# sahaRatul/sela

Hardware: NVIDIA H100
Metric: encode+decode MSamples/s (higher is better)
Workload: dtype f64+int64

## Files before the change

### sela_b200/csrc/c_abi.cu

```cuda
#include <algorithm>
#include <atomic>
#include <cstdarg>
#include <cstdio>
#include <cstdlib>
#include <cstring>
#include <mutex>
#include <thread>
#include <vector>

#include "lossless.cuh"
#include "verify.cuh"

using namespace selab200;

namespace {

thread_local char g_error[512] = "";
std::mutex g_mutex;
std::atomic<uint64_t> g_launches{0};

int fail(int code, const char *fmt, ...)
{
    va_list ap;
    va_start(ap, fmt);
// ... 217 lines not shown
    const std::pair<const void *, int> key(reinterpret_cast<const void *>(kernel), dev);
    std::lock_guard<std::mutex> lock(m);
    for (auto &e : done)
        if (e.first == key) {
            if (e.second >= bytes)
                return 0;
            CUDA_TRY(cudaFuncSetAttribute(kernel, cudaFuncAttributeMaxDynamicSharedMemorySize, (int)bytes));
            e.second = bytes;
            return 0;
        }
    CUDA_TRY(cudaFuncSetAttribute(kernel, cudaFuncAttributeMaxDynamicSharedMemorySize, (int)bytes));
    done.emplace_back(key, bytes);
    return 0;
}

int launch_check(const char *what)
{
    g_launches.fetch_add(1, std::memory_order_relaxed);
    cudaError_t e = cudaGetLastError();
    if (e != cudaSuccess)
        return fail(SELAB200_ERR_CUDA, "launch of %s failed: %s", what, cudaGetErrorString(e));
    return 0;
}

template <int KIND>
int launch_unit_means(const void *src, size_t n_units, uint32_t channels, double *means, cudaStream_t stream)
{
    const MeanTiling mt = mean_tiling(KIND, channels);
    k_unit_means<KIND><<<(unsigned)((n_units + 31) / 32), 32, unit_means_smem_bytes(mt), stream>>>(src, (uint32_t)n_units,
                                                                                                 channels, means);
    return launch_check("k_unit_means");
}

template <bool STEREO, bool TRACE, bool CHECK = false, bool FORCE = false>
int launch_encode_units(const EncodeParams &p, size_t n_units, selab200_analysis_trace *d_trace, cudaStream_t stream,
                        const selab200_predictor *d_pred = nullptr)
{
    constexpr size_t smem = encode_smem_bytes<STEREO>();
    if (int rc = set_smem(k_encode_units<STEREO, TRACE, CHECK, FORCE>, smem))
        return rc;
    k_encode_units<STEREO, TRACE, CHECK, FORCE><<<(unsigned)n_units, 32, smem, stream>>>(p, d_trace, d_pred);
    return launch_check("k_encode_units");
}

template <bool STEREO, bool FORCE = false>
int launch_repair(const EncodeParams &p, const RepairParams &r, size_t n_frames, size_t n_units, cudaStream_t stream,
                  const selab200_predictor *d_pred = nullptr)
{
    constexpr size_t smem = encode_smem_bytes<STEREO>();
    if (int rc = set_smem(k_lossless_candidates<STEREO, FORCE>, smem))
        return rc;
    if (int rc = set_smem(k_lossless_repack<STEREO, FORCE>, smem))
        return rc;
    k_lossless_select<<<(unsigned)((n_frames + 255) / 256), 256, 0, stream>>>(p, r);
    if (int rc = launch_check("k_lossless_select"))
        return rc;
    const unsigned warps = (unsigned)std::min(n_units, (size_t)g.sms * 32);
    for (int round = 0; round < 2; round++) {
        k_lossless_candidates<STEREO, FORCE><<<warps, 32, smem, stream>>>(p, r, round, d_pred);
        if (int rc = launch_check("k_lossless_candidates"))
            return rc;
    }
    k_lossless_repack<STEREO, FORCE><<<warps, 32, smem, stream>>>(p, r, d_pred);
    if (int rc = launch_check("k_lossless_repack"))
        return rc;
    k_lossless_report<<<(unsigned)std::min((n_frames + 255) / 256, (size_t)g.sms), 256, 0, stream>>>(p, r);
// ... 21 lines not shown

int encode_device(const int16_t *d_pcm, uint32_t n_frames, uint32_t channels, selab200_subframe_desc *d_descs,
                  uint32_t *d_words, size_t capacity, uint64_t *d_used, int32_t *d_status, void *d_ws,
                  size_t ws_bytes, cudaStream_t stream, const EncodeOptions &o = EncodeOptions())
{
    if (int rc = check_channels(channels))
        return rc;
    if (ws_bytes < (o.lossless ? selab200_encode_lossless_workspace_bytes(n_frames, channels)
                               : selab200_encode_workspace_bytes(n_frames, channels)))
        return fail(SELAB200_ERR_ARGUMENT, "encode workspace too small");
    if (channels == 2 && (reinterpret_cast<uintptr_t>(d_pcm) & 15) != 0)
        return fail(SELAB200_ERR_ARGUMENT, "stereo PCM must be 16-byte aligned on the device");
    if (o.fresh) {
        CUDA_TRY(cudaMemsetAsync(d_status, 0, sizeof(int32_t), stream));
        CUDA_TRY(cudaMemsetAsync(d_used, 0, sizeof(uint64_t), stream));
    }
    if (n_frames == 0)
        return 0;
    const bool stereo = channels == 2;
    const size_t n_units = encode_units(n_frames, channels);
    const size_t n_sub = (size_t)n_frames * channels;
    EncodeParams p;
    p.pcm = d_pcm;
    p.n_frames = n_frames;
    p.channels = channels;
    p.descs = d_descs;
    p.words = d_words;
    p.capacity = capacity;
    p.words_used = reinterpret_cast<unsigned long long *>(d_used);
    p.status = d_status;
    p.units = static_cast<UnitRecord *>(d_ws);
    p.slots = reinterpret_cast<uint32_t *>(static_cast<char *>(d_ws) + align256(n_units * sizeof(UnitRecord)));
    p.means = reinterpret_cast<double *>(reinterpret_cast<char *>(p.slots) + align256(n_units * (size_t)kSlotWords * 4));
    p.residues = reinterpret_cast<int32_t *>(reinterpret_cast<char *>(p.means) + align256(n_units * sizeof(double)));
    if (int rc = stereo ? launch_unit_means<kMeanStereo>(d_pcm, n_units, channels, p.means, stream)
                        : launch_unit_means<kMeanPcm>(d_pcm, n_units, channels, p.means, stream))
        return rc;
    if (o.lossless) {
        RepairParams r;
        char *b = static_cast<char *>(d_ws) + align256(selab200_encode_workspace_bytes(n_frames, channels));
        r.count = reinterpret_cast<uint32_t *>(b);
        r.frames = reinterpret_cast<uint32_t *>(b + 256);
        r.orig = reinterpret_cast<UnitRecord *>(b + 256 + align256((size_t)n_frames * 4));
        r.units = reinterpret_cast<RepairUnit *>(reinterpret_cast<char *>(r.orig) + align256(n_units * sizeof(UnitRecord)));
        r.entries = o.lossless->entries;
        r.n_entries = o.lossless->n_entries;
        r.frame_base = o.lossless->frame_base;
        CUDA_TRY(cudaMemsetAsync(r.count, 0, 2 * sizeof(uint32_t), stream));
        if (o.d_pred) {
            if (int rc = stereo ? launch_encode_units<true, false, true, true>(p, n_units, nullptr, stream, o.d_pred)
                                : launch_encode_units<false, false, true, true>(p, n_units, nullptr, stream, o.d_pred))
                return rc;
            if (int rc = stereo ? launch_repair<true, true>(p, r, n_frames, n_units, stream, o.d_pred)
                                : launch_repair<false, true>(p, r, n_frames, n_units, stream, o.d_pred))
                return rc;
        } else {
            if (int rc = stereo ? launch_encode_units<true, false, true>(p, n_units, nullptr, stream)
                                : launch_encode_units<false, false, true>(p, n_units, nullptr, stream))
                return rc;
            if (int rc = stereo ? launch_repair<true>(p, r, n_frames, n_units, stream)
                                : launch_repair<false>(p, r, n_frames, n_units, stream))
                return rc;
        }
    } else {
        const int rc_units = stereo ? (o.d_trace ? launch_encode_units<true, true>(p, n_units, o.d_trace, stream)
                                                 : launch_encode_units<true, false>(p, n_units, nullptr, stream))
                                    : (o.d_trace ? launch_encode_units<false, true>(p, n_units, o.d_trace, stream)
                                                 : launch_encode_units<false, false>(p, n_units, nullptr, stream));
        if (rc_units)
// ... 398 lines not shown
}

void selab200_shutdown(void)
{
    std::lock_guard<std::mutex> lock(g_mutex);
    shutdown_all();
}

void *selab200_host_alloc(size_t bytes)
{
    void *p = nullptr;
    if (cudaMallocHost(&p, bytes ? bytes : 1) != cudaSuccess) {
        fail(SELAB200_ERR_CUDA, "cudaMallocHost(%zu) failed", bytes);
        return nullptr;
    }
    return p;
}

void selab200_host_free(void *p)
{
    if (p)
        cudaFreeHost(p);
}

size_t selab200_encode_words_bound(uint32_t n_frames, uint32_t channels)
{
    return (size_t)n_frames * channels * kSlotWords + 64;
}

size_t selab200_encode_workspace_bytes(uint32_t n_frames, uint32_t channels)
{
    const size_t n_units = encode_units(n_frames, channels);
    return align256(n_units * sizeof(UnitRecord)) + align256(n_units * (size_t)kSlotWords * 4) +
           align256(n_units * sizeof(double)) + n_units * (size_t)kFrame * 4 + 256;
}

size_t selab200_encode_lossless_workspace_bytes(uint32_t n_frames, uint32_t channels)
{
    return align256(selab200_encode_workspace_bytes(n_frames, channels)) + repair_lists_bytes(n_frames, channels);
}

size_t selab200_decode_workspace_bytes(uint32_t n_frames, uint32_t channels)
{
    const size_t n_sub = (size_t)n_frames * channels;
    return align256(n_sub * 128 * 4) + align256(n_sub * kFrame * 4) + align256(synthesis_warps(n_sub) * 32 * 4) +
           align256(n_sub * 64) + 256;
}

size_t selab200_verify_workspace_bytes(uint32_t n_frames, uint32_t channels)
{
    return align256(selab200_decode_workspace_bytes(n_frames, channels)) + align256((size_t)n_frames * channels * kFrame * 2);
}

int selab200_encode_frames_device(const int16_t *d_pcm, uint32_t n_frames, uint32_t channels,
                                  selab200_subframe_desc *d_descs, uint32_t *d_words, size_t words_capacity,
                                  uint64_t *d_words_used, int32_t *d_status, void *d_workspace,
                                  size_t workspace_bytes, void *stream)
{
    std::lock_guard<std::mutex> lock(g_mutex);
    if (int rc = d_pcm ? require_ready_for(d_pcm) : require_ready())
        return rc;
    if (!d_pcm || !d_descs || !d_words || !d_words_used || !d_status || !d_workspace)
        return fail(SELAB200_ERR_ARGUMENT, "null device pointer");
    return encode_device(d_pcm, n_frames, channels, d_descs, d_words, words_capacity, d_words_used, d_status,
                         d_workspace, workspace_bytes, (cudaStream_t)stream);
}

// ... 1170 lines not shown
                       int32_t *residues)
{
    std::lock_guard<std::mutex> lock(g_mutex);
    return fir_probe(samples, orders, c, n, wide, residues, nullptr);
}

int selab200_fir_tie_probe(const int32_t *samples, const int32_t *orders, const int64_t *c, uint32_t n, int wide,
                           int32_t *residues, uint8_t *ties)
{
    std::lock_guard<std::mutex> lock(g_mutex);
    if (int rc = require_ready())
        return rc;
    if (!ties)
        return fail(SELAB200_ERR_ARGUMENT, "null pointer");
    return fir_probe(samples, orders, c, n, wide, residues, ties);
}


int selab200_lpc_residues(const int32_t *samples, uint32_t n_sub, uint8_t *order, int32_t *q, int32_t *residues)
{
    std::lock_guard<std::mutex> lock(g_mutex);
    if (int rc = require_ready())
        return rc;
    if (!samples || !order || !q || !residues)
        return fail(SELAB200_ERR_ARGUMENT, "null pointer");
    if (n_sub == 0)
        return 0;
    for (size_t i = 0; i < (size_t)n_sub * kFrame; i++)
        if (samples[i] > 65535 || samples[i] < -65535)
            return fail(SELAB200_ERR_RANGE, "sample %zu = %d outside the 17-bit domain of 16-bit audio", i, samples[i]);
    const size_t sig = (size_t)n_sub * kFrame * 4;
    if (int rc = g.in.ensure(sig)) return rc;
    if (int rc = g.work.ensure(sig)) return rc;
    if (int rc = g.aux.ensure(align256((size_t)n_sub * sizeof(double)) + (size_t)n_sub * kMaxOrder * 4 + n_sub + 256)) return rc;
    double *d_means = static_cast<double *>(g.aux.ptr);
    int32_t *d_q = reinterpret_cast<int32_t *>(static_cast<char *>(g.aux.ptr) + align256((size_t)n_sub * sizeof(double)));
    uint8_t *d_order = reinterpret_cast<uint8_t *>(d_q + (size_t)n_sub * kMaxOrder);
    CUDA_TRY(cudaMemcpyAsync(g.in.ptr, samples, sig, cudaMemcpyHostToDevice, g.stream));
    if (int rc = launch_unit_means<kMeanPlanar>(g.in.ptr, n_sub, 1, d_means, g.stream))
        return rc;
    k_lpc_residues<<<n_sub, 32, 0, g.stream>>>(static_cast<const int32_t *>(g.in.ptr), d_means, n_sub, d_order, d_q,
                                               static_cast<int32_t *>(g.work.ptr));
    if (int rc = launch_check("k_lpc_residues"))
        return rc;
    CUDA_TRY(cudaMemcpyAsync(residues, g.work.ptr, sig, cudaMemcpyDeviceToHost, g.stream));
    CUDA_TRY(cudaMemcpyAsync(q, d_q, (size_t)n_sub * kMaxOrder * 4, cudaMemcpyDeviceToHost, g.stream));
    CUDA_TRY(cudaMemcpyAsync(order, d_order, n_sub, cudaMemcpyDeviceToHost, g.stream));
    CUDA_TRY(cudaStreamSynchronize(g.stream));
    return 0;
}

int selab200_lpc_samples(const int32_t *residues, uint32_t n_sub, const uint8_t *order, const int32_t *q,
                         int32_t *samples)
{
    std::lock_guard<std::mutex> lock(g_mutex);
    if (int rc = require_ready())
        return rc;
    if (!residues || !order || !q || !samples)
        return fail(SELAB200_ERR_ARGUMENT, "null pointer");
    if (n_sub == 0)
        return 0;
    for (uint32_t i = 0; i < n_sub; i++)
        if (order[i] > kMaxOrder)
            return fail(SELAB200_ERR_BITSTREAM, "order[%u] = %u exceeds %d", i, order[i], kMaxOrder);
    const size_t sig = (size_t)n_sub * kFrame * 4;
    if (int rc = g.in.ensure(sig)) return rc;
    if (int rc = g.work.ensure(sig)) return rc;
    if (int rc = g.aux.ensure((size_t)n_sub * kMaxOrder * 4 + n_sub + 256)) return rc;
    int32_t *d_q = static_cast<int32_t *>(g.aux.ptr);
    uint8_t *d_order = reinterpret_cast<uint8_t *>(d_q + (size_t)n_sub * kMaxOrder);
    CUDA_TRY(cudaMemcpyAsync(g.in.ptr, residues, sig, cudaMemcpyHostToDevice, g.stream));
    CUDA_TRY(cudaMemcpyAsync(d_q, q, (size_t)n_sub * kMaxOrder * 4, cudaMemcpyHostToDevice, g.stream));
    CUDA_TRY(cudaMemcpyAsync(d_order, order, n_sub, cudaMemcpyHostToDevice, g.stream));
    k_lpc_samples<<<n_sub, 32, 0, g.stream>>>(static_cast<const int32_t *>(g.in.ptr), n_sub, d_order, d_q,
// ... 81 lines not shown
```

### sela_b200/csrc/kernels.cuh

```cuda
#pragma once

#include "lpc.cuh"
#include "rice.cuh"
#include "rice_vs.cuh"

namespace selab200 {

enum { kMeanPcm = 0, kMeanStereo = 1, kMeanPlanar = 2 };
constexpr int kMeanTile = 64;
constexpr int kMeanSlots = 16;

struct MeanTiling {
    uint32_t units_per_row;
    uint32_t step;
    uint32_t row_stride;
    uint32_t rows_max;
    uint32_t row_words;
};

__host__ __device__ inline MeanTiling mean_tiling(int kind, uint32_t channels)
{
    MeanTiling t;
    uint32_t span = 1;
    if (kind == kMeanPcm) {
// ... 53 lines not shown
        __syncwarp();
#pragma unroll
        for (int s = 0; s < kMeanSlots; s++)
            if (lane + 32 * s < total) {
                staged[soff[s]] = buf[s].x;
                staged[soff[s] + 1] = buf[s].y;
                staged[soff[s] + 2] = buf[s].z;
                staged[soff[s] + 3] = buf[s].w;
            }
        __syncwarp();
        if (t + 1 < kFrame / kMeanTile)
            fetch(t + 1);
#pragma unroll 8
        for (int j = 0; j < kMeanTile; j++) {
            int x;
            if (KIND == kMeanPcm) {
                x = *reinterpret_cast<const int16_t *>(at + j * mt.step);
            } else if (KIND == kMeanStereo) {
                const uint32_t pair = *reinterpret_cast<const uint32_t *>(at + 4 * j);
                const int a = (int)(pair << 16) >> 16, b = (int)pair >> 16;
                x = role == 0 ? a : role == 1 ? b : a - b;
            } else {
                x = *reinterpret_cast<const int32_t *>(at + 4 * j);
            }
            chain.add(x);
        }
    }
    if (u < n_units)
        means[u] = chain.mean();
}

inline size_t unit_means_smem_bytes(const MeanTiling &mt) { return (size_t)mt.rows_max * mt.row_words * 4; }


constexpr uint32_t kSlotWords = 1600;
constexpr uint32_t kSlotReflWords = 32;

struct __align__(16) UnitRecord {
    uint32_t order;
    uint32_t refl_k, refl_words;
    uint32_t res_k, res_words;
    uint32_t flags;
    uint32_t pad[2];
};

struct EncodeParams {
    const int16_t *pcm;
    uint32_t n_frames, channels;
    selab200_subframe_desc *descs;
    uint32_t *words;
    unsigned long long capacity;
    unsigned long long *words_used;
    int32_t *status;
    UnitRecord *units;
    uint32_t *slots;
    double *means;
    int32_t *residues;
};

__host__ __device__ inline uint32_t encode_units(uint32_t n_frames, uint32_t channels)
{
    return channels == 2 ? n_frames * 3u : n_frames * channels;
}

struct PredictorEdit {
    int order, j, delta;
};
__host__ __device__ inline int repair_round1(int o) { return o == 2 ? 5 : 7; }
__host__ __device__ inline int repair_candidates(int o) { return o < 2 ? 0 : 3 * o - 1; }
constexpr int kRepairRound2Max = 3 * kMaxOrder - 1 - 7;
__host__ __device__ inline PredictorEdit repair_edit(int o, int c)
{
    PredictorEdit e{o, 0, 0};
    const int n1 = repair_round1(o);
    if (c < n1) {
        if (c == n1 - 1) {
            e.order = o - 1;
        } else {
            e.j = (c >> 1) < 2 ? (c >> 1) : o - 1;
            e.delta = (c & 1) ? 1 : -1;
        }
        return e;
    }
    c -= n1;
    const int n_edits = o > 3 ? 2 * (o - 3) : 0;
    if (c < n_edits) {
        e.j = 2 + (c >> 1);
        e.delta = (c & 1) ? 1 : -1;
    } else {
        e.order = o - 2 - (c - n_edits);
    }
    return e;
}

struct RepairUnit {
    uint32_t unit, order;
    unsigned long long best;
};
constexpr unsigned long long kNoCandidate = ~0ull;

enum { kUnitEncode = 0, kUnitCheck = 1, kUnitCandidate = 2, kUnitRepack = 3 };

template <bool STEREO, bool TRACE, int MODE, bool FORCE = false>
__device__ __forceinline__ void encode_unit(const EncodeParams &p, selab200_analysis_trace *trace, const uint32_t unit,
                                            RepairUnit *ru, uint32_t cand, const selab200_predictor *pred = nullptr)
{
    constexpr int kRow = kHistoryPad + kFrame;
    constexpr int kLoWords = (kHistoryPad + kFrame) / 32;
    extern __shared__ __align__(16) unsigned char smem_raw[];
    int16_t *s16 = reinterpret_cast<int16_t *>(smem_raw);
    uint32_t *lo_bits = reinterpret_cast<uint32_t *>(smem_raw + kRow * 2);
    constexpr size_t kSigBytes = kRow * 2 + (STEREO ? kLoWords * 4 : 0);
    AnalysisScratch &scratch = *reinterpret_cast<AnalysisScratch *>(smem_raw + kSigBytes);
    static_assert(kCoefAlias + sizeof(CoefSmem) <= sizeof(AnalysisScratch) && kCoefAlias % 16 == 0, "predictor alias");
    CoefSmem &cf = *reinterpret_cast<CoefSmem *>(smem_raw + kSigBytes + kCoefAlias);

    const int lane = lane_id();
    const uint32_t frame = STEREO ? unit / 3 : unit / p.channels;
    const uint32_t role = STEREO ? unit % 3 : unit % p.channels;

    const int16_t *src = p.pcm + (size_t)frame * kFrame * p.channels;
    for (int j = lane; j < kHistoryPad / 2; j += 32)
        reinterpret_cast<uint32_t *>(s16)[j] = 0;
    int16_t *row = s16 + kHistoryPad;
    Signal sig;
    sig.a = row;
    sig.lo = nullptr;
    if (STEREO) {
        const uint4 *src128 = reinterpret_cast<const uint4 *>(src);
        if (role < 2) {
            const uint32_t sel = role ? 0x7632 : 0x5410;
            for (int j = lane; j < kFrame / 4; j += 32) {
                const uint4 v = src128[j];
                reinterpret_cast<uint2 *>(row)[j] = make_uint2(__byte_perm(v.x, v.y, sel), __byte_perm(v.z, v.w, sel));
            }
        } else {
            if (lane < kHistoryPad / 32)
                lo_bits[lane] = 0;
            uint32_t *lo = lo_bits + kHistoryPad / 32;
            for (int it = 0; it < kFrame / 128; it++) {
                const uint4 v = src128[it * 32 + lane];
                const uint32_t pr[4] = {v.x, v.y, v.z, v.w};
                int d[4];
#pragma unroll
                for (int e = 0; e < 4; e++)
                    d[e] = ((int)(pr[e] << 16) >> 16) - ((int)pr[e] >> 16);
                const uint32_t h01 = ((uint32_t)(d[0] >> 1) & 0xffffu) | ((uint32_t)(d[1] >> 1) << 16);
                const uint32_t h23 = ((uint32_t)(d[2] >> 1) & 0xffffu) | ((uint32_t)(d[3] >> 1) << 16);
                reinterpret_cast<uint2 *>(row)[it * 32 + lane] = make_uint2(h01, h23);
                uint32_t nib = (d[0] & 1) | ((d[1] & 1) << 1) | ((d[2] & 1) << 2) | ((d[3] & 1) << 3);
                nib <<= 4 * (lane & 7);
                nib |= __shfl_xor_sync(kFull, nib, 1);
                nib |= __shfl_xor_sync(kFull, nib, 2);
                nib |= __shfl_xor_sync(kFull, nib, 4);
                if ((lane & 7) == 0)
                    lo[it * 4 + (lane >> 3)] = nib;
            }
            sig.lo = lo;
        }
    } else {
        for (int j = lane; j < kFrame; j += 32)
            row[j] = src[(size_t)j * p.channels + role];
    }
    __syncwarp();

    int32_t *res = p.residues + (size_t)(MODE == kUnitEncode || MODE == kUnitCheck ? unit : blockIdx.x) * kFrame;
    warp_autocorrelation(sig, scratch, shfl_d(lane == 0 ? p.means[unit] : 0.0, 0));
    if constexpr (TRACE) {
        selab200_analysis_trace &tr = trace[unit];
        if (lane == 0)
            tr.mean = p.means[unit];
        for (int i = lane; i <= kMaxOrder; i += 32)
            tr.ac[i] = scratch.ac[i];
    }
    warp_schur(scratch);
    int order = warp_order_and_quantise(scratch, cf);
    if constexpr (FORCE) {
        const selab200_predictor &f = pred[unit];
        for (int i = lane; i < kMaxOrder; i += 32)
            cf.q[i] = f.q[i];
        order = f.order;
        __syncwarp();
    }
    if constexpr (MODE == kUnitCandidate || MODE == kUnitRepack) {
        const PredictorEdit e = repair_edit(order, (int)cand);
        if (e.delta) {
            const int v = cf.q[e.j] + e.delta;
            if (v < -64 || v > 63)
                return;
            __syncwarp();
            if (lane == 0)
                cf.q[e.j] = v;
        } else {
            for (int i = e.order + lane; i < order; i += 32)
                cf.q[i] = 0;
        }
        __syncwarp();
        order = e.order;
    }
    warp_coefficients(cf, scratch.t(), order);
    if constexpr (TRACE) {
        selab200_analysis_trace &tr = trace[unit];
        for (int i = lane; i < kMaxOrder; i += 32) {
            tr.k[i] = scratch.kk()[i];
            tr.q[i] = cf.q[i];
        }
        for (int i = lane; i <= kMaxOrder; i += 32)
            tr.c[i] = i == 0 ? 0 : coef_at(cf, i);
        if (lane == 0)
            tr.order = order;
    }
    static_assert(kPlaneBytes <= kCoefAlias, "FIR digit planes");
    uint32_t *planes = reinterpret_cast<uint32_t *>(scratch.ring);
    constexpr bool kCheck = MODE == kUnitCheck || MODE == kUnitCandidate;
    bool tie;
    if (STEREO && role == 2)
        tie = warp_fir_residual<true, kCheck>(sig, cf, order, planes, res);
    else
        tie = warp_fir_residual<false, kCheck>(sig, cf, order, planes, res);

    const RiceChoice cq = warp_rice_choose(cf.q, order);
    const RiceChoice cr = warp_rice_choose(res, kFrame);
    if constexpr (MODE == kUnitCandidate) {
        __syncwarp();
        for (int l = lane; l < kFrame * 4 / 128; l += 32)
            asm volatile("discard.global.L2 [%0], 128;" ::"l"(res + l * 32) : "memory");
        const unsigned long long round = cand >= (uint32_t)repair_round1(ru->order) ? 1ull : 0ull;
        if (lane == 0 && !tie)
            atomicMin(&ru->best, round << 63 | (unsigned long long)(cq.words + cr.words) << 32 | cand);
        return;
    }
    const bool too_large = cq.words > kSlotReflWords || cr.words > kSlotWords - kSlotReflWords;
    uint32_t *slot = p.slots + (size_t)unit * kSlotWords;
    if (!too_large) {
        warp_rice_pack(cf.q, order, cq, slot);
        warp_rice_pack(res, kFrame, cr, slot + kSlotReflWords);
    }
    __syncwarp();
    for (int l = lane; l < kFrame * 4 / 128; l += 32)
        asm volatile("discard.global.L2 [%0], 128;" ::"l"(res + l * 32) : "memory");
    if (lane == 0) {
        UnitRecord u;
        u.order = order;
        u.refl_k = cq.k;
        u.refl_words = cq.words;
        u.res_k = cr.k;
// ... 563 lines not shown
    for (uint32_t pos = 0; pos < ch; pos++)
        any |= fd[pos].subframe_type == 1;
    if (!any || !frame_check(fd, ch, p.n_words))
        return;
    int16_t *out = p.pcm_out + (size_t)frame * kFrame * ch;
    for (uint32_t pos = 0; pos < ch; pos++) {
        const selab200_subframe_desc d = fd[pos];
        if (d.subframe_type != 1)
            continue;
        const int32_t *diff = p.ws_res + ((size_t)frame * ch + pos) * kFrame;
        for (int t = threadIdx.x; t < kFrame; t += blockDim.x)
            out[(size_t)t * ch + d.channel] =
                (int16_t)(uint16_t)((uint32_t)out[(size_t)t * ch + d.parent_channel] - (uint32_t)diff[t]);
    }
}


struct Row17 {
    __align__(16) int16_t a[kHistoryPad + kFrame];
    uint32_t lo[(kHistoryPad + kFrame) / 32];
    __device__ __forceinline__ Signal stage(const int32_t *src)
    {
        const int lane = lane_id();
        for (int i = lane; i < kHistoryPad / 2; i += 32)
            reinterpret_cast<uint32_t *>(a)[i] = 0;
        if (lane < kHistoryPad / 32)
            lo[lane] = 0;
        stage_17bit_row(src, a + kHistoryPad, lo + kHistoryPad / 32);
        __syncwarp();
        return Signal{a + kHistoryPad, lo + kHistoryPad / 32};
    }
};

__global__ void __launch_bounds__(32) k_lpc_residues(const int32_t *samples, const double *means, uint32_t n_sub,
                                                     uint8_t *order_out, int32_t *q_out, int32_t *residues)
{
    __shared__ __align__(16) AnalysisScratch scratch;
    __shared__ __align__(16) CoefSmem cf;
    __shared__ __align__(16) Row17 row;
    const uint32_t sub = blockIdx.x;
    const int lane = lane_id();
    const Signal sig = row.stage(samples + (size_t)sub * kFrame);
    warp_autocorrelation(sig, scratch, means[sub]);
    warp_schur(scratch);
    const int order = warp_order_and_quantise(scratch, cf);
    warp_coefficients(cf, scratch.t(), order);
    warp_fir_residual<true>(sig, cf, order, reinterpret_cast<uint32_t *>(scratch.ring), residues + (size_t)sub * kFrame);
    for (int i = lane; i < kMaxOrder; i += 32)
        q_out[(size_t)sub * kMaxOrder + i] = i < order ? cf.q[i] : 0;
    if (lane == 0)
        order_out[sub] = (uint8_t)order;
}

template <bool CHECK = false>
__global__ void __launch_bounds__(32) k_fir_probe(const int32_t *samples, const int32_t *orders, const long long *c,
                                                  int wide, int32_t *residues, uint8_t *ties)
{
    __shared__ __align__(16) AnalysisScratch scratch;
    __shared__ __align__(16) CoefSmem cf;
    __shared__ __align__(16) Row17 row;
    const uint32_t sub = blockIdx.x;
    const int lane = lane_id();
    const int32_t *src = samples + (size_t)sub * kFrame;
    Signal sig = row.stage(src);
    if (!wide) {
        for (int j = lane; j < kFrame; j += 32)
            row.a[kHistoryPad + j] = (int16_t)src[j];
        sig.lo = nullptr;
    }
    const int order = orders[sub];
    for (int i = lane; i < 112; i += 32) {
        const long long v = i < order ? c[(size_t)sub * (kMaxOrder + 1) + i + 1] : 0;
        cf.clo[i] = (uint32_t)v;
        cf.chi[i] = (int32_t)(v >> 32);
    }
    __syncwarp();
    uint32_t *planes = reinterpret_cast<uint32_t *>(scratch.ring);
    int32_t *res = residues + (size_t)sub * kFrame;
    const bool tie = wide ? warp_fir_residual<true, CHECK>(sig, cf, order, planes, res)
                          : warp_fir_residual<false, CHECK>(sig, cf, order, planes, res);
    if (CHECK && lane == 0)
        ties[sub] = tie;
}

__global__ void __launch_bounds__(32) k_lpc_samples(const int32_t *residues, uint32_t n_sub, const uint8_t *order_in,
                                                    const int32_t *q_in, int32_t *samples)
{
    __shared__ __align__(16) SegSmem sm;
    const uint32_t sub = blockIdx.x;
    const int lane = lane_id();
    const int order = min((int)order_in[sub], kMaxOrder);
    const int n = segment_width(order);
    if (lane == 0) {
        sm.row_res[0] = residues + (size_t)sub * kFrame;
        sm.row_out[0] = samples + (size_t)sub * kFrame;
        sm.row_mode[0] = 2;
    }
    __syncwarp();
    segment_synthesis(sm, 0, lane, n, 0, 1, lane < n ? order : 0, q_in + (size_t)sub * kMaxOrder, 1);
}

__global__ void k_quantise_probe(const double *k, uint32_t n, int32_t *out)
{
    const uint32_t i = blockIdx.x * blockDim.x + threadIdx.x;
    if (i >= n)
        return;
    const double kv = k[i];
    out[4 * (size_t)i + 0] = quantise_reflection(0, kv);
    out[4 * (size_t)i + 1] = quantise_reflection(1, kv);
    out[4 * (size_t)i + 2] = quantise_reflection(2, kv);
// ... 60 lines not shown
```

### sela_b200/csrc/lpc.cuh

```cuda
#pragma once

#include "common.cuh"
#include "lpc_tables.cuh"

namespace selab200 {

struct CoefSmem {
    uint32_t clo[112];
    int32_t  chi[112];
    int32_t  q[104];
};
struct AnalysisScratch {
    double ring[256];
    double ac[128];
    __device__ __forceinline__ double *kk() { return ring; }
    __device__ __forceinline__ double *t() { return ring + 104; }
};
using LpcSmem = AnalysisScratch;
constexpr size_t kCoefAlias = 208 * sizeof(double);

__device__ __forceinline__ long long coef_at(const CoefSmem &cf, int j)
{
    return (long long)(((unsigned long long)(uint32_t)cf.chi[j - 1] << 32) | cf.clo[j - 1]);
}

__device__ __forceinline__ int ring_chunk(int chunk)
{
    chunk &= 127;
    return chunk ^ ((chunk >> 3) & 1);
}
__device__ __forceinline__ int ring_index(int p)
{
    return (ring_chunk(p >> 1) << 1) | (p & 1);
}

__device__ __forceinline__ double sample_to_x(int s)
{
    const double rcp = 1.0 / 32767.0;
    const double a = (double)s;
    const double q0 = __dmul_rn(a, rcp);
    const double r = __fma_rn(-q0, 32767.0, a);
    return __fma_rn(r, rcp, q0);
}
__device__ __forceinline__ double sample_to_x_div(int s) { return ddiv((double)s, 32767.0); }

struct MeanChain {
    double sum = 0.0;
    __device__ __forceinline__ void add(int s) { sum = dadd(sum, sample_to_x(s)); }
    __device__ __forceinline__ double mean() const { return ddiv(sum, (double)kFrame); }
};

template <typename Sig>
__device__ void warp_autocorrelation(const Sig &sig, LpcSmem &sm, const double mean)
{
    const int lane = lane_id();

    {
        double2 *r2 = reinterpret_cast<double2 *>(sm.ring);
        r2[64 + lane] = make_double2(0.0, 0.0);
        r2[96 + lane] = make_double2(0.0, 0.0);
    }
    double acc0 = 0.0, acc1 = 0.0, acc2 = 0.0, acc3 = 0.0;
    double p1 = 0.0, p2 = 0.0, p3 = 0.0;
    const char *ringb = reinterpret_cast<const char *>(sm.ring);
    int own_off[8];
#pragma unroll
    for (int i = 0; i < 8; i++) {
        const int rel = i - lane;
        own_off[i] = 16 * (2 * rel + ((rel >> 2) & 1));
    }

    for (int tile = 0; tile < kFrame / 128; tile++) {
        __syncwarp();
#pragma unroll
        for (int r = 0; r < 4; r++) {
            int j = tile * 128 + r * 32 + lane;
            sm.ring[ring_index(j)] = dsub(sample_to_x(sig.at(j)), mean);
        }
        __syncwarp();
        for (int blk = 0; blk < 4; blk++) {
            const int gb = (tile * 32 + blk * 8) * 32;
            const char *bbase = ringb + (gb & 2047);
#pragma unroll
            for (int i = 0; i < 8; i++) {
                const int oo = (gb + own_off[i]) & 2047;
                const double2 o0 = *reinterpret_cast<const double2 *>(ringb + oo);
                const double2 o1 = *reinterpret_cast<const double2 *>(ringb + (oo ^ 16));
                constexpr int kSw[8] = {0, 0, 0, 0, 16, 16, 16, 16};
                const double2 b0 = *reinterpret_cast<const double2 *>(bbase + ((32 * i) ^ kSw[i]));
                const double2 b1 = *reinterpret_cast<const double2 *>(bbase + ((32 * i + 16) ^ kSw[i]));
                const double c0 = o0.x, c1 = o0.y, c2 = o1.x, c3 = o1.y;
                acc0 = dadd(acc0, dmul(b0.x, c0));
                acc1 = dadd(acc1, dmul(b0.x, p1));
                acc2 = dadd(acc2, dmul(b0.x, p2));
                acc3 = dadd(acc3, dmul(b0.x, p3));
                acc0 = dadd(acc0, dmul(b0.y, c1));
                acc1 = dadd(acc1, dmul(b0.y, c0));
                acc2 = dadd(acc2, dmul(b0.y, p1));
                acc3 = dadd(acc3, dmul(b0.y, p2));
                acc0 = dadd(acc0, dmul(b1.x, c2));
                acc1 = dadd(acc1, dmul(b1.x, c1));
                acc2 = dadd(acc2, dmul(b1.x, c0));
                acc3 = dadd(acc3, dmul(b1.x, p1));
                acc0 = dadd(acc0, dmul(b1.y, c3));
                acc1 = dadd(acc1, dmul(b1.y, c2));
                acc2 = dadd(acc2, dmul(b1.y, c1));
                acc3 = dadd(acc3, dmul(b1.y, c0));
                p1 = c3;
                p2 = c2;
                p3 = c1;
            }
        }
    }
    __syncwarp();
    sm.ac[4 * lane + 0] = acc0;
    sm.ac[4 * lane + 1] = acc1;
    sm.ac[4 * lane + 2] = acc2;
    sm.ac[4 * lane + 3] = acc3;
    __syncwarp();
    const double ac0 = sm.ac[0];
    __syncwarp();
#pragma unroll
    for (int t = 0; t < 4; t++) {
        int i = lane + 32 * t;
        if (i >= 1 && i <= kMaxOrder)
            sm.ac[i] = ddiv(sm.ac[i], ac0);
    }
    if (lane == 0)
        sm.ac[0] = 1.0;
    __syncwarp();
}

__device__ void warp_schur(LpcSmem &sm)
{
    const int lane = lane_id();
    double *kk = sm.kk();
    double g0[4], g1[4];
#pragma unroll
    for (int m = 0; m < 4; m++) {
        int j = 4 * lane + m;
        double v = (j < kMaxOrder) ? sm.ac[j + 1] : 0.0;
        g0[m] = v;
        g1[m] = v;
    }
    double err = sm.ac[0];
    double head = shfl_d(g1[0], 0);
    double k = ddiv(-head, err);
    err = dadd(err, dmul(head, k));
    if (lane == 0)
        kk[0] = k;
    for (int i = 1; i < kMaxOrder; i++) {
        const double kp = k;
        const double nxt = shfl_down_d(g1[0], 1);
        double up[4] = {g1[1], g1[2], g1[3], nxt};
#pragma unroll
        for (int m = 0; m < 4; m++) {
            double n1 = dadd(up[m], dmul(kp, g0[m]));
            double n0 = dadd(dmul(up[m], kp), g0[m]);
            g1[m] = n1;
            g0[m] = n0;
        }
        head = shfl_d(g1[0], 0);
        k = ddiv(-head, err);
        err = dadd(err, dmul(head, k));
        if (lane == 0)
            kk[i] = k;
    }
    __syncwarp();
}


__device__ __forceinline__ bool reflection_significant(double kv) { return fabs(kv) > 0.05; }

__device__ __forceinline__ int quantise_reflection(int i, double kv)
{
    const double sqrt2 = 1.4142135623730950488016887242096;
    double v;
    if (i == 0)
        v = floor(dmul(64.0, dadd(-1.0, dmul(sqrt2, dsqrt(dadd(kv, 1.0))))));
    else if (i == 1)
        v = floor(dmul(64.0, dadd(-1.0, dmul(sqrt2, dsqrt(dadd(-kv, 1.0))))));
    else
        v = floor(dmul(64.0, kv));
    return isnan(v) ? 0 : __double2int_rz(v);
}

__device__ int warp_order_and_quantise(LpcSmem &sm, CoefSmem &cf)
{
    const int lane = lane_id();
    const double *kk = sm.kk();
    int best = -1;
#pragma unroll
    for (int t = 0; t < 4; t++) {
        int i = lane + 32 * t;
        if (i < kMaxOrder && reflection_significant(kk[i]))
            best = i;
    }
    best = __reduce_max_sync(kFull, best);
    const int order = best < 0 ? 1 : best + 1;

#pragma unroll
    for (int t = 0; t < 4; t++) {
        int i = lane + 32 * t;
        if (i < order) {
            cf.q[i] = quantise_reflection(i, kk[i]);
        } else if (i < 104) {
            cf.q[i] = 0;
        }
    }
    __syncwarp();
    return order;
}

__device__ __forceinline__ double dequantise(int i, int q)
{
    int idx = q + 64;
    idx = idx < 0 ? 0 : (idx > 127 ? 127 : idx);
    if (i == 0)
        return __longlong_as_double((long long)selab200_FIRST_BITS[idx]);
    if (i == 1)
        return idx == 0 ? __longlong_as_double((long long)SELAB200_SECOND0_BITS)
                        : -__longlong_as_double((long long)selab200_FIRST_BITS[idx]);
    return (double)(idx - 64) / 64.0;
// ... 5 lines not shown
    for (int i = lane; i < 112; i += 32) {
        cf.clo[i] = 0;
        cf.chi[i] = 0;
    }
    __syncwarp();
    if (order <= 1)
        return;
    for (int i = 0; i < order; i++) {
        const double ki = dequantise(i, cf.q[i]);
        const int half = i >> 1;
        for (int j = lane; j < half; j += 32) {
            double a = t[j];
            double b = t[i - 1 - j];
            t[j] = dadd(a, dmul(ki, b));
            t[i - 1 - j] = dadd(b, dmul(ki, a));
        }
        if (lane == 0) {
            if (i & 1) {
                double mid = t[half];
                t[half] = dadd(mid, dmul(mid, ki));
            }
            t[i] = ki;
        }
        __syncwarp();
    }
    const double scale = 34359738368.0;
    for (int m = lane; m < order; m += 32) {
        const long long v = __double2ll_rz(dmul(scale, -t[m]));
        cf.clo[m] = (uint32_t)v;
        cf.chi[m] = (int32_t)(v >> 32);
    }
    __syncwarp();
}

constexpr int kPlaneWords = 34;
constexpr size_t kPlaneBytes = 8 * kPlaneWords * 4;

__device__ int warp_fir_planes(const CoefSmem &cf, uint32_t *planes)
{
    const unsigned long long H = 0x8080808080808080ull;
    const int lane = lane_id();
    __syncwarp();
    int nd = 0;
    for (int w = lane; w < kPlaneWords; w += 32) {
        unsigned long long e[4];
#pragma unroll
        for (int i = 0; i < 4; i++) {
            const int j = 4 * w + i - 7;
            const unsigned long long c = (j >= 1 && j <= 112) ? (unsigned long long)coef_at(cf, j) : 0ull;
            e[i] = (c + H) ^ H;
            nd = max(nd, (64 - __clzll((long long)e[i]) + 7) >> 3);
        }
#pragma unroll
        for (int p = 0; p < 8; p++) {
            uint32_t v = 0;
#pragma unroll
            for (int i = 0; i < 4; i++)
                v |= (uint32_t)((e[i] >> (8 * p)) & 0xffu) << (8 * i);
            planes[p * kPlaneWords + w] = v;
        }
    }
    __syncwarp();
    return __reduce_max_sync(kFull, nd);
}

__device__ __forceinline__ uint32_t prmt(uint32_t x, uint32_t y, uint32_t sel)
{
    uint32_t d;
    asm("prmt.b32 %0, %1, %2, %3;" : "=r"(d) : "r"(x), "r"(y), "r"(sel));
// ... 301 lines not shown
```

Before: 12910.

## Compute per-unit autocorrelation in a dedicated multi-unit warp kernel

Moves the LPC autocorrelation out of the per-unit encode warp into a new kernel that processes four units per warp, with eight lanes per unit each holding thirteen lag accumulators over a shared-memory sliding window. The normalised autocorrelation is written to a global workspace, and Schur recursion reads it from there. The analysis scratch is also shrunk to a union of kk, t and the FIR planes, plus the coefficient struct, which lowers shared memory per block. The trade-off is an extra kernel launch and a global round trip for the autocorrelation rows, and the FP accumulation order changes, which could alter the predictors chosen.

New measurement: 13430, median of 6. +4.0%, better.

```diff
diff --git a/sela_b200/csrc/c_abi.cu b/sela_b200/csrc/c_abi.cu
--- a/sela_b200/csrc/c_abi.cu
+++ b/sela_b200/csrc/c_abi.cu
@@ -273,6 +273,15 @@
     return launch_check("k_unit_means");
 }
 
+template <int KIND>
+int launch_unit_autocorrelation(const void *src, size_t n_units, uint32_t channels, const double *means, double *ac,
+                                cudaStream_t stream)
+{
+    const unsigned warps = (unsigned)((n_units + kAcUnitsPerWarp - 1) / kAcUnitsPerWarp);
+    k_unit_autocorrelation<KIND><<<warps, 32, 0, stream>>>(src, (uint32_t)n_units, channels, means, ac);
+    return launch_check("k_unit_autocorrelation");
+}
+
 template <bool STEREO, bool TRACE, bool CHECK = false, bool FORCE = false>
 int launch_encode_units(const EncodeParams &p, size_t n_units, selab200_analysis_trace *d_trace, cudaStream_t stream,
                         const selab200_predictor *d_pred = nullptr)
@@ -360,9 +369,14 @@
     p.units = static_cast<UnitRecord *>(d_ws);
     p.slots = reinterpret_cast<uint32_t *>(static_cast<char *>(d_ws) + align256(n_units * sizeof(UnitRecord)));
     p.means = reinterpret_cast<double *>(reinterpret_cast<char *>(p.slots) + align256(n_units * (size_t)kSlotWords * 4));
-    p.residues = reinterpret_cast<int32_t *>(reinterpret_cast<char *>(p.means) + align256(n_units * sizeof(double)));
+    p.ac = reinterpret_cast<double *>(reinterpret_cast<char *>(p.means) + align256(n_units * sizeof(double)));
+    p.residues = reinterpret_cast<int32_t *>(reinterpret_cast<char *>(p.ac) + align256(n_units * kAcPitch * sizeof(double)));
     if (int rc = stereo ? launch_unit_means<kMeanStereo>(d_pcm, n_units, channels, p.means, stream)
                         : launch_unit_means<kMeanPcm>(d_pcm, n_units, channels, p.means, stream))
+        return rc;
+
+    if (int rc = stereo ? launch_unit_autocorrelation<kMeanStereo>(d_pcm, n_units, channels, p.means, p.ac, stream)
+                        : launch_unit_autocorrelation<kMeanPcm>(d_pcm, n_units, channels, p.means, p.ac, stream))
         return rc;
     if (o.lossless) {
         RepairParams r;
@@ -827,7 +841,8 @@
 {
     const size_t n_units = encode_units(n_frames, channels);
     return align256(n_units * sizeof(UnitRecord)) + align256(n_units * (size_t)kSlotWords * 4) +
-           align256(n_units * sizeof(double)) + n_units * (size_t)kFrame * 4 + 256;
+           align256(n_units * sizeof(double)) + align256(n_units * kAcPitch * sizeof(double)) +
+           n_units * (size_t)kFrame * 4 + 256;
 }
 
 size_t selab200_encode_lossless_workspace_bytes(uint32_t n_frames, uint32_t channels)
@@ -2064,14 +2079,19 @@
     const size_t sig = (size_t)n_sub * kFrame * 4;
     if (int rc = g.in.ensure(sig)) return rc;
     if (int rc = g.work.ensure(sig)) return rc;
-    if (int rc = g.aux.ensure(align256((size_t)n_sub * sizeof(double)) + (size_t)n_sub * kMaxOrder * 4 + n_sub + 256)) return rc;
+    const size_t ac_bytes = align256((size_t)n_sub * kAcPitch * sizeof(double));
+    if (int rc = g.aux.ensure(align256((size_t)n_sub * sizeof(double)) + ac_bytes + (size_t)n_sub * kMaxOrder * 4 + n_sub + 256))
+        return rc;
     double *d_means = static_cast<double *>(g.aux.ptr);
-    int32_t *d_q = reinterpret_cast<int32_t *>(static_cast<char *>(g.aux.ptr) + align256((size_t)n_sub * sizeof(double)));
+    double *d_ac = reinterpret_cast<double *>(static_cast<char *>(g.aux.ptr) + align256((size_t)n_sub * sizeof(double)));
+    int32_t *d_q = reinterpret_cast<int32_t *>(reinterpret_cast<char *>(d_ac) + ac_bytes);
     uint8_t *d_order = reinterpret_cast<uint8_t *>(d_q + (size_t)n_sub * kMaxOrder);
     CUDA_TRY(cudaMemcpyAsync(g.in.ptr, samples, sig, cudaMemcpyHostToDevice, g.stream));
     if (int rc = launch_unit_means<kMeanPlanar>(g.in.ptr, n_sub, 1, d_means, g.stream))
         return rc;
-    k_lpc_residues<<<n_sub, 32, 0, g.stream>>>(static_cast<const int32_t *>(g.in.ptr), d_means, n_sub, d_order, d_q,
+    if (int rc = launch_unit_autocorrelation<kMeanPlanar>(g.in.ptr, n_sub, 1, d_means, d_ac, g.stream))
+        return rc;
+    k_lpc_residues<<<n_sub, 32, 0, g.stream>>>(static_cast<const int32_t *>(g.in.ptr), d_ac, n_sub, d_order, d_q,
                                                static_cast<int32_t *>(g.work.ptr));
     if (int rc = launch_check("k_lpc_residues"))
         return rc;
diff --git a/sela_b200/csrc/kernels.cuh b/sela_b200/csrc/kernels.cuh
--- a/sela_b200/csrc/kernels.cuh
+++ b/sela_b200/csrc/kernels.cuh
@@ -109,6 +109,85 @@
 
 inline size_t unit_means_smem_bytes(const MeanTiling &mt) { return (size_t)mt.rows_max * mt.row_words * 4; }
 
+template <int KIND>
+__device__ __forceinline__ int unit_sample(const void *src, uint32_t channels, uint32_t u, int j)
+{
+    if (KIND == kMeanPcm)
+        return static_cast<const int16_t *>(src)[((size_t)(u / channels) * kFrame + j) * channels + u % channels];
+    if (KIND == kMeanStereo) {
+        const uint32_t pair = static_cast<const uint32_t *>(src)[(size_t)(u / 3) * kFrame + j];
+        const int a = (int)(pair << 16) >> 16, b = (int)pair >> 16, role = u % 3;
+        return role == 0 ? a : role == 1 ? b : a - b;
+    }
+    return static_cast<const int32_t *>(src)[(size_t)u * kFrame + j];
+}
+
+template <int KIND>
+__global__ void __launch_bounds__(32) k_unit_autocorrelation(const void *src, uint32_t n_units,
+                                                             uint32_t channels, const double *means, double *ac)
+{
+    __shared__ __align__(16) double rows[kAcUnitsPerWarp * kAcRow];
+    const int lane = lane_id(), grp = lane / kAcLanesPerUnit, k = lane % kAcLanesPerUnit;
+    const uint32_t first = blockIdx.x * kAcUnitsPerWarp;
+    const uint32_t mine = min(first + grp, n_units - 1);
+    const double mean = means[mine];
+
+    for (int i = lane; i < kAcUnitsPerWarp * kAcRow; i += 32)
+        rows[i] = 0.0;
+    const double *own = rows + grp * kAcRow + kAcHist;
+    double acc[kAcLagsPerLane], w[kAcLagsPerLane];
+#pragma unroll
+    for (int m = 0; m < kAcLagsPerLane; m++)
+        acc[m] = w[m] = 0.0;
+    for (int j0 = kAcFirst; j0 < kFrame; j0 += kAcTile) {
+        __syncwarp();
+        if (j0 != kAcFirst) {
+            constexpr int kPer = kAcUnitsPerWarp * kAcHist / 2 / 32;
+            double2 h[kPer];
+#pragma unroll
+            for (int r = 0; r < kPer; r++) {
+                const int v = lane + 32 * r, g = v / (kAcHist / 2), i = 2 * (v % (kAcHist / 2));
+                h[r] = *reinterpret_cast<const double2 *>(rows + g * kAcRow + kAcTile + i);
+            }
+#pragma unroll
+            for (int r = 0; r < kPer; r++) {
+                const int v = lane + 32 * r, g = v / (kAcHist / 2), i = 2 * (v % (kAcHist / 2));
+                *reinterpret_cast<double2 *>(rows + g * kAcRow + i) = h[r];
+            }
+        }
+#pragma unroll
+        for (int g = 0; g < kAcUnitsPerWarp; g++) {
+            const uint32_t u = min(first + g, n_units - 1);
+            const double mu = shfl_d(mean, g * kAcLanesPerUnit);
+            for (int jj = lane; jj < kAcTile; jj += 32) {
+                const int j = j0 + jj;
+                rows[g * kAcRow + kAcHist + jj] = j < 0 ? 0.0 : dsub(sample_to_x(unit_sample<KIND>(src, channels, u, j)), mu);
+            }
+        }
+        __syncwarp();
+        const double *wb = own - kAcLagsPerLane * k;
+        for (int s = 0; s < kAcTile; s += kAcLagsPerLane) {
+#pragma unroll
+            for (int t = 0; t < kAcLagsPerLane; t++) {
+                const double b = own[s + t];
+                w[t] = wb[s + t];
+#pragma unroll
+                for (int m = 0; m < kAcLagsPerLane; m++)
+                    acc[m] = dadd(acc[m], dmul(b, w[(t - m + kAcLagsPerLane) % kAcLagsPerLane]));
+            }
+        }
+    }
+    const double ac0 = shfl_d(acc[0], grp * kAcLanesPerUnit);
+    if (first + grp >= n_units)
+        return;
+    double *row = ac + (size_t)(first + grp) * kAcPitch + kAcLagsPerLane * k;
+#pragma unroll
+    for (int m = 0; m < kAcLagsPerLane; m++) {
+        const int i = kAcLagsPerLane * k + m;
+        row[m] = i == 0 ? 1.0 : i <= kMaxOrder ? ddiv(acc[m], ac0) : 0.0;
+    }
+}
+
 
 constexpr uint32_t kSlotWords = 1600;
 constexpr uint32_t kSlotReflWords = 32;
@@ -132,6 +211,7 @@
     UnitRecord *units;
     uint32_t *slots;
     double *means;
+    double *ac;
     int32_t *residues;
 };
 
@@ -189,8 +269,7 @@
     uint32_t *lo_bits = reinterpret_cast<uint32_t *>(smem_raw + kRow * 2);
     constexpr size_t kSigBytes = kRow * 2 + (STEREO ? kLoWords * 4 : 0);
     AnalysisScratch &scratch = *reinterpret_cast<AnalysisScratch *>(smem_raw + kSigBytes);
-    static_assert(kCoefAlias + sizeof(CoefSmem) <= sizeof(AnalysisScratch) && kCoefAlias % 16 == 0, "predictor alias");
-    CoefSmem &cf = *reinterpret_cast<CoefSmem *>(smem_raw + kSigBytes + kCoefAlias);
+    CoefSmem &cf = scratch.cf;
 
     const int lane = lane_id();
     const uint32_t frame = STEREO ? unit / 3 : unit / p.channels;
@@ -242,16 +321,18 @@
     __syncwarp();
 
     int32_t *res = p.residues + (size_t)(MODE == kUnitEncode || MODE == kUnitCheck ? unit : blockIdx.x) * kFrame;
-    warp_autocorrelation(sig, scratch, shfl_d(lane == 0 ? p.means[unit] : 0.0, 0));
+    const double *ac = p.ac + (size_t)unit * kAcPitch;
+    warp_schur(ac, scratch.kk);
+    int order = warp_order_and_quantise(scratch.kk, cf);
     if constexpr (TRACE) {
         selab200_analysis_trace &tr = trace[unit];
         if (lane == 0)
             tr.mean = p.means[unit];
         for (int i = lane; i <= kMaxOrder; i += 32)
-            tr.ac[i] = scratch.ac[i];
-    }
-    warp_schur(scratch);
-    int order = warp_order_and_quantise(scratch, cf);
+            tr.ac[i] = ac[i];
+        for (int i = lane; i < kMaxOrder; i += 32)
+            tr.k[i] = scratch.kk[i];
+    }
     if constexpr (FORCE) {
         const selab200_predictor &f = pred[unit];
         for (int i = lane; i < kMaxOrder; i += 32)
@@ -275,20 +356,17 @@
         __syncwarp();
         order = e.order;
     }
-    warp_coefficients(cf, scratch.t(), order);
+    warp_coefficients(cf, scratch.t, order);
     if constexpr (TRACE) {
         selab200_analysis_trace &tr = trace[unit];
-        for (int i = lane; i < kMaxOrder; i += 32) {
-            tr.k[i] = scratch.kk()[i];
+        for (int i = lane; i < kMaxOrder; i += 32)
             tr.q[i] = cf.q[i];
-        }
         for (int i = lane; i <= kMaxOrder; i += 32)
             tr.c[i] = i == 0 ? 0 : coef_at(cf, i);
         if (lane == 0)
             tr.order = order;
     }
-    static_assert(kPlaneBytes <= kCoefAlias, "FIR digit planes");
-    uint32_t *planes = reinterpret_cast<uint32_t *>(scratch.ring);
+    uint32_t *planes = scratch.planes;
     constexpr bool kCheck = MODE == kUnitCheck || MODE == kUnitCandidate;
     bool tie;
     if (STEREO && role == 2)
@@ -918,20 +996,19 @@
     }
 };
 
-__global__ void __launch_bounds__(32) k_lpc_residues(const int32_t *samples, const double *means, uint32_t n_sub,
+__global__ void __launch_bounds__(32) k_lpc_residues(const int32_t *samples, const double *ac, uint32_t n_sub,
                                                      uint8_t *order_out, int32_t *q_out, int32_t *residues)
 {
     __shared__ __align__(16) AnalysisScratch scratch;
-    __shared__ __align__(16) CoefSmem cf;
     __shared__ __align__(16) Row17 row;
+    CoefSmem &cf = scratch.cf;
     const uint32_t sub = blockIdx.x;
     const int lane = lane_id();
     const Signal sig = row.stage(samples + (size_t)sub * kFrame);
-    warp_autocorrelation(sig, scratch, means[sub]);
-    warp_schur(scratch);
-    const int order = warp_order_and_quantise(scratch, cf);
-    warp_coefficients(cf, scratch.t(), order);
-    warp_fir_residual<true>(sig, cf, order, reinterpret_cast<uint32_t *>(scratch.ring), residues + (size_t)sub * kFrame);
+    warp_schur(ac + (size_t)sub * kAcPitch, scratch.kk);
+    const int order = warp_order_and_quantise(scratch.kk, cf);
+    warp_coefficients(cf, scratch.t, order);
+    warp_fir_residual<true>(sig, cf, order, scratch.planes, residues + (size_t)sub * kFrame);
     for (int i = lane; i < kMaxOrder; i += 32)
         q_out[(size_t)sub * kMaxOrder + i] = i < order ? cf.q[i] : 0;
     if (lane == 0)
@@ -943,8 +1020,8 @@
                                                   int wide, int32_t *residues, uint8_t *ties)
 {
     __shared__ __align__(16) AnalysisScratch scratch;
-    __shared__ __align__(16) CoefSmem cf;
     __shared__ __align__(16) Row17 row;
+    CoefSmem &cf = scratch.cf;
     const uint32_t sub = blockIdx.x;
     const int lane = lane_id();
     const int32_t *src = samples + (size_t)sub * kFrame;
@@ -961,7 +1038,7 @@
         cf.chi[i] = (int32_t)(v >> 32);
     }
     __syncwarp();
-    uint32_t *planes = reinterpret_cast<uint32_t *>(scratch.ring);
+    uint32_t *planes = scratch.planes;
     int32_t *res = residues + (size_t)sub * kFrame;
     const bool tie = wide ? warp_fir_residual<true, CHECK>(sig, cf, order, planes, res)
                           : warp_fir_residual<false, CHECK>(sig, cf, order, planes, res);
diff --git a/sela_b200/csrc/lpc.cuh b/sela_b200/csrc/lpc.cuh
--- a/sela_b200/csrc/lpc.cuh
+++ b/sela_b200/csrc/lpc.cuh
@@ -10,28 +10,21 @@
     int32_t  chi[112];
     int32_t  q[104];
 };
+constexpr int kPlaneWords = 34;
+constexpr size_t kPlaneBytes = 8 * kPlaneWords * 4;
+
 struct AnalysisScratch {
-    double ring[256];
-    double ac[128];
-    __device__ __forceinline__ double *kk() { return ring; }
-    __device__ __forceinline__ double *t() { return ring + 104; }
+    union {
+        double kk[104];
+        double t[104];
+        uint32_t planes[8 * kPlaneWords];
+    };
+    CoefSmem cf;
 };
-using LpcSmem = AnalysisScratch;
-constexpr size_t kCoefAlias = 208 * sizeof(double);
 
 __device__ __forceinline__ long long coef_at(const CoefSmem &cf, int j)
 {
     return (long long)(((unsigned long long)(uint32_t)cf.chi[j - 1] << 32) | cf.clo[j - 1]);
-}
-
-__device__ __forceinline__ int ring_chunk(int chunk)
-{
-    chunk &= 127;
-    return chunk ^ ((chunk >> 3) & 1);
-}
-__device__ __forceinline__ int ring_index(int p)
-{
-    return (ring_chunk(p >> 1) << 1) | (p & 1);
 }
 
 __device__ __forceinline__ double sample_to_x(int s)
@@ -50,100 +43,29 @@
     __device__ __forceinline__ double mean() const { return ddiv(sum, (double)kFrame); }
 };
 
-template <typename Sig>
-__device__ void warp_autocorrelation(const Sig &sig, LpcSmem &sm, const double mean)
+constexpr int kAcLagsPerLane = 13;
+constexpr int kAcLanesPerUnit = 8;
+constexpr int kAcUnitsPerWarp = 32 / kAcLanesPerUnit;
+constexpr int kAcPitch = kAcLagsPerLane * kAcLanesPerUnit;
+constexpr int kAcTile = 8 * kAcLagsPerLane;
+constexpr int kAcFirst = kFrame - (kFrame + kAcTile - 1) / kAcTile * kAcTile;
+constexpr int kAcHist = 96;
+constexpr int kAcRow = kAcHist + kAcTile;
+static_assert(kAcPitch > kMaxOrder && kAcHist >= kAcLagsPerLane * (kAcLanesPerUnit - 1) && kAcHist % 2 == 0 &&
+                  kAcTile >= kAcHist && kAcRow % 16 == 8, "autocorrelation layout");
+
+__device__ void warp_schur(const double *ac, double *kk)
 {
     const int lane = lane_id();
-
-    {
-        double2 *r2 = reinterpret_cast<double2 *>(sm.ring);
-        r2[64 + lane] = make_double2(0.0, 0.0);
-        r2[96 + lane] = make_double2(0.0, 0.0);
-    }
-    double acc0 = 0.0, acc1 = 0.0, acc2 = 0.0, acc3 = 0.0;
-    double p1 = 0.0, p2 = 0.0, p3 = 0.0;
-    const char *ringb = reinterpret_cast<const char *>(sm.ring);
-    int own_off[8];
-#pragma unroll
-    for (int i = 0; i < 8; i++) {
-        const int rel = i - lane;
-        own_off[i] = 16 * (2 * rel + ((rel >> 2) & 1));
-    }
-
-    for (int tile = 0; tile < kFrame / 128; tile++) {
-        __syncwarp();
-#pragma unroll
-        for (int r = 0; r < 4; r++) {
-            int j = tile * 128 + r * 32 + lane;
-            sm.ring[ring_index(j)] = dsub(sample_to_x(sig.at(j)), mean);
-        }
-        __syncwarp();
-        for (int blk = 0; blk < 4; blk++) {
-            const int gb = (tile * 32 + blk * 8) * 32;
-            const char *bbase = ringb + (gb & 2047);
-#pragma unroll
-            for (int i = 0; i < 8; i++) {
-                const int oo = (gb + own_off[i]) & 2047;
-                const double2 o0 = *reinterpret_cast<const double2 *>(ringb + oo);
-                const double2 o1 = *reinterpret_cast<const double2 *>(ringb + (oo ^ 16));
-                constexpr int kSw[8] = {0, 0, 0, 0, 16, 16, 16, 16};
-                const double2 b0 = *reinterpret_cast<const double2 *>(bbase + ((32 * i) ^ kSw[i]));
-                const double2 b1 = *reinterpret_cast<const double2 *>(bbase + ((32 * i + 16) ^ kSw[i]));
-                const double c0 = o0.x, c1 = o0.y, c2 = o1.x, c3 = o1.y;
-                acc0 = dadd(acc0, dmul(b0.x, c0));
-                acc1 = dadd(acc1, dmul(b0.x, p1));
-                acc2 = dadd(acc2, dmul(b0.x, p2));
-                acc3 = dadd(acc3, dmul(b0.x, p3));
-                acc0 = dadd(acc0, dmul(b0.y, c1));
-                acc1 = dadd(acc1, dmul(b0.y, c0));
-                acc2 = dadd(acc2, dmul(b0.y, p1));
-                acc3 = dadd(acc3, dmul(b0.y, p2));
-                acc0 = dadd(acc0, dmul(b1.x, c2));
-                acc1 = dadd(acc1, dmul(b1.x, c1));
-                acc2 = dadd(acc2, dmul(b1.x, c0));
-                acc3 = dadd(acc3, dmul(b1.x, p1));
-                acc0 = dadd(acc0, dmul(b1.y, c3));
-                acc1 = dadd(acc1, dmul(b1.y, c2));
-                acc2 = dadd(acc2, dmul(b1.y, c1));
-                acc3 = dadd(acc3, dmul(b1.y, c0));
-                p1 = c3;
-                p2 = c2;
-                p3 = c1;
-            }
-        }
-    }
-    __syncwarp();
-    sm.ac[4 * lane + 0] = acc0;
-    sm.ac[4 * lane + 1] = acc1;
-    sm.ac[4 * lane + 2] = acc2;
-    sm.ac[4 * lane + 3] = acc3;
-    __syncwarp();
-    const double ac0 = sm.ac[0];
-    __syncwarp();
-#pragma unroll
-    for (int t = 0; t < 4; t++) {
-        int i = lane + 32 * t;
-        if (i >= 1 && i <= kMaxOrder)
-            sm.ac[i] = ddiv(sm.ac[i], ac0);
-    }
-    if (lane == 0)
-        sm.ac[0] = 1.0;
-    __syncwarp();
-}
-
-__device__ void warp_schur(LpcSmem &sm)
-{
-    const int lane = lane_id();
-    double *kk = sm.kk();
     double g0[4], g1[4];
 #pragma unroll
     for (int m = 0; m < 4; m++) {
         int j = 4 * lane + m;
-        double v = (j < kMaxOrder) ? sm.ac[j + 1] : 0.0;
+        double v = (j < kMaxOrder) ? ac[j + 1] : 0.0;
         g0[m] = v;
         g1[m] = v;
     }
-    double err = sm.ac[0];
+    double err = ac[0];
     double head = shfl_d(g1[0], 0);
     double k = ddiv(-head, err);
     err = dadd(err, dmul(head, k));
@@ -185,10 +107,9 @@
     return isnan(v) ? 0 : __double2int_rz(v);
 }
 
-__device__ int warp_order_and_quantise(LpcSmem &sm, CoefSmem &cf)
+__device__ int warp_order_and_quantise(const double *kk, CoefSmem &cf)
 {
     const int lane = lane_id();
-    const double *kk = sm.kk();
     int best = -1;
 #pragma unroll
     for (int t = 0; t < 4; t++) {
@@ -260,9 +181,6 @@
     }
     __syncwarp();
 }
-
-constexpr int kPlaneWords = 34;
-constexpr size_t kPlaneBytes = 8 * kPlaneWords * 4;
 
 __device__ int warp_fir_planes(const CoefSmem &cf, uint32_t *planes)
 {
```
